# kwea123/ngp_pl

Measured on AMD Instinct MI355X. Metric: train rays/sec (800x800 Lego-like, 8192 rays/batch/GPU, full step incl. optimizer), higher is better.
Workload: dtype f16/f32

## Files before the change

### ngp_pl_amd/_lib.py

```python
import contextlib
import ctypes as C
import os

import torch

_HERE = os.path.dirname(os.path.abspath(__file__))
LIB_PATH = os.environ.get("NGP_HIP_LIB") or os.path.join(_HERE, "csrc", "libngp_hip.so")

P = C.c_void_p
I = C.c_int
F = C.c_float
L = C.c_int64

NGP_MAX_LEVELS = 16


class GridMeta(C.Structure):
    _fields_ = [("n_levels", C.c_int32), ("n_features", C.c_int32),
                ("offset", C.c_uint32 * (NGP_MAX_LEVELS + 1)),
                ("resolution", C.c_uint32 * NGP_MAX_LEVELS),
                ("scale", C.c_float * NGP_MAX_LEVELS)]


class StepperConfig(C.Structure):
# ... 209 lines not shown


def call(name, *args):
    rc = getattr(lib(), name)(*args)
    if name in _COUNT_QUERIES:
        return rc
    if rc != 0:
        kind = {-1: "NGP_EINVAL (bad argument)", -2: "NGP_EUNSUP (unsupported configuration)",
                -3: "NGP_ETIMEOUT (a device result did not arrive within NGP_SPIN_TIMEOUT_S)"}.get(rc, "hipError_t %d" % rc)
        if rc == -4:
            kind = "NGP_ECOMM (%s)" % (lib().ngp_comm_last_error() or b"?").decode(errors="replace")
        raise NgpError("%s failed: %s" % (name, kind))
    return 0


_FIELD_BWD_USES_H = None


def field_bwd_uses_h():
    global _FIELD_BWD_USES_H
    if _FIELD_BWD_USES_H is None:
        _FIELD_BWD_USES_H = bool(call("ngp_field_bwd_uses_h"))
    return _FIELD_BWD_USES_H


SPIN_TIMEOUT_S = float(os.environ.get("NGP_SPIN_TIMEOUT_S", "30"))


class DeviceTimeout(NgpError):
    """A host poll on a device result ran out of time: the kernel named in the message did not finish."""
# ... 77 lines not shown
```

### ngp_pl_amd/build.py

```python
import os
import subprocess
import sys
from concurrent.futures import ThreadPoolExecutor

HERE = os.path.dirname(os.path.abspath(__file__))
CSRC = os.path.join(HERE, "csrc")
LIB = os.path.join(CSRC, "libngp_hip.so")
SOURCES = ["march.hip", "composite.hip", "hashgrid.hip", "mlp.hip", "optim.hip", "occupancy.hip", "hashgrid_bwd_binned.hip", "stepper.hip", "comm.hip"]
HEADERS = ["ngp_common.h", "hashgrid_common.h", "loss_common.h", "comm.h", "adam_common.h", os.path.join("..", "..", "include", "ngp_hip.h")]
ARCH = "gfx950"
HIPCC = os.environ.get("HIPCC", "/opt/rocm/bin/hipcc")
CFLAGS = ["--offload-arch=" + ARCH, "-O3", "-std=c++17", "-fPIC", "-fvisibility=hidden",
          "-fhip-fp32-correctly-rounded-divide-sqrt", "-Wno-unused-result"]
EXTRA = {"mlp.hip": ["-mllvm", "-amdgpu-mfma-vgpr-form"]}
MESH_LIB = os.path.join(CSRC, "libngp_mesh.so")
MESH_SOURCES = [os.path.join("mesh", "mesh.hip")]
MESH_HEADERS = [os.path.join("mesh", "mc_tables.h"), os.path.join("..", "..", "include", "ngp_mesh.h")]
MESH_CFLAGS = ["-ffp-contract=off"]
MESHFILTER_LIB = os.path.join(CSRC, "libngp_meshfilter.so")
MESHFILTER_SOURCES = [os.path.join("meshfilter", "meshfilter.hip")]
MESHFILTER_HEADERS = ["mesh_compact.h", os.path.join("..", "..", "include", "ngp_meshfilter.h")]
MESHCULL_LIB = os.path.join(CSRC, "libngp_meshcull.so")
MESHCULL_SOURCES = [os.path.join("meshcull", "meshcull.hip")]
MESHCULL_HEADERS = ["mesh_compact.h", "mesh_camera.h", "mesh_raster.h", os.path.join("..", "..", "include", "ngp_meshcull.h")]
MESHCULL_CFLAGS = ["-ffp-contract=off"]
MESHSIMPLIFY_LIB = os.path.join(CSRC, "libngp_meshsimplify.so")
MESHSIMPLIFY_SOURCES = [os.path.join("meshsimplify", "meshsimplify.hip")]
MESHSIMPLIFY_HEADERS = ["mesh_compact.h", os.path.join("..", "..", "include", "ngp_meshsimplify.h")]
MESHSIMPLIFY_CFLAGS = ["-ffp-contract=off"]
# ... 55 lines not shown

def _plan(sources, headers, extra, force):
    hdrs = [os.path.join(CSRC, h) for h in headers]
    objs, jobs = [], []
    for src in sources:
        s = os.path.join(CSRC, src)
        o = os.path.join(CSRC, src.replace(".hip", ".o"))
        objs.append(o)
        if force or _stale(o, [s, os.path.abspath(__file__)] + hdrs):
            jobs.append([HIPCC] + CFLAGS + extra(src) + ["-c", s, "-o", o])
    return objs, jobs


def build(force=False, verbose=False):
    objs, jobs = _plan(SOURCES, HEADERS, lambda src: EXTRA.get(src, []), force)
    mesh_objs, mesh_jobs = _plan(MESH_SOURCES, MESH_HEADERS, lambda src: MESH_CFLAGS, force)
    filter_objs, filter_jobs = _plan(MESHFILTER_SOURCES, MESHFILTER_HEADERS, lambda src: [], force)
    cull_objs, cull_jobs = _plan(MESHCULL_SOURCES, MESHCULL_HEADERS, lambda src: MESHCULL_CFLAGS, force)
    simplify_objs, simplify_jobs = _plan(MESHSIMPLIFY_SOURCES, MESHSIMPLIFY_HEADERS, lambda src: MESHSIMPLIFY_CFLAGS, force)
    tsdf_objs, tsdf_jobs = _plan(MESHTSDF_SOURCES, MESHTSDF_HEADERS, lambda src: MESHTSDF_CFLAGS, force)
    smooth_objs, smooth_jobs = _plan(MESHSMOOTH_SOURCES, MESHSMOOTH_HEADERS, lambda src: MESHSMOOTH_CFLAGS, force)
    tex_objs, tex_jobs = _plan(MESHTEX_SOURCES, MESHTEX_HEADERS, lambda src: MESHTEX_CFLAGS, force)
    metrics_objs, metrics_jobs = _plan(METRICS_SOURCES, METRICS_HEADERS, lambda src: METRICS_CFLAGS, force)
    dist_objs, dist_jobs = _plan(MESHDIST_SOURCES, MESHDIST_HEADERS, lambda src: MESHDIST_CFLAGS, force)
    quadric_objs, quadric_jobs = _plan(MESHQUADRIC_SOURCES, MESHQUADRIC_HEADERS, lambda src: MESHQUADRIC_CFLAGS, force)
    decimate_objs, decimate_jobs = _plan(MESHDECIMATE_SOURCES, MESHDECIMATE_HEADERS, lambda src: MESHDECIMATE_CFLAGS, force)
    atlas_objs, atlas_jobs = _plan(MESHATLAS_SOURCES, MESHATLAS_HEADERS, lambda src: MESHATLAS_CFLAGS, force)
    photo_objs, photo_jobs = _plan(MESHPHOTO_SOURCES, MESHPHOTO_HEADERS, lambda src: MESHPHOTO_CFLAGS, force)
    normal_objs, normal_jobs = _plan(MESHNORMAL_SOURCES, MESHNORMAL_HEADERS, lambda src: MESHNORMAL_CFLAGS, force)
    todo = (jobs + mesh_jobs + filter_jobs + cull_jobs + simplify_jobs + tsdf_jobs + smooth_jobs + tex_jobs + metrics_jobs + dist_jobs
            + quadric_jobs + decimate_jobs + atlas_jobs + photo_jobs + normal_jobs)
    if todo:
        if verbose:
            print("[ngp_pl_amd.build] compiling %d HIP sources for %s" % (len(todo), ARCH))
        with ThreadPoolExecutor(max_workers=min(len(todo), os.cpu_count() or 1)) as ex:
            list(ex.map(_run, todo))
    for lib, o, changed in ((LIB, objs, jobs), (MESH_LIB, mesh_objs, mesh_jobs), (MESHFILTER_LIB, filter_objs, filter_jobs),
                            (MESHCULL_LIB, cull_objs, cull_jobs), (MESHSIMPLIFY_LIB, simplify_objs, simplify_jobs),
                            (MESHTSDF_LIB, tsdf_objs, tsdf_jobs), (MESHSMOOTH_LIB, smooth_objs, smooth_jobs),
                            (MESHTEX_LIB, tex_objs, tex_jobs), (METRICS_LIB, metrics_objs, metrics_jobs),
                            (MESHDIST_LIB, dist_objs, dist_jobs), (MESHQUADRIC_LIB, quadric_objs, quadric_jobs),
                            (MESHDECIMATE_LIB, decimate_objs, decimate_jobs), (MESHATLAS_LIB, atlas_objs, atlas_jobs),
                            (MESHPHOTO_LIB, photo_objs, photo_jobs), (MESHNORMAL_LIB, normal_objs, normal_jobs)):
        if force or changed or _stale(lib, o):
            _run([HIPCC, "--offload-arch=" + ARCH, "-shared", "-fPIC"] + o + ["-o", lib])
            if verbose:
                print("[ngp_pl_amd.build] linked", lib)
    return LIB


if __name__ == "__main__":
    build(force="--force" in sys.argv, verbose=True)
# ... 1 lines not shown
```

### ngp_pl_amd/csrc/composite.hip

```cpp
#pragma clang fp contract(off)

#include "ngp_common.h"
#include "loss_common.h"

namespace {

__device__ __forceinline__ float wave_incl_prod(float v, int lane) {
#pragma unroll
    for (int o = 1; o < 64; o <<= 1) { const float u = __shfl_up(v, o, 64); if (lane >= o) v *= u; }
    return v;
}
__device__ __forceinline__ float wave_incl_sum(float v, int lane) {
#pragma unroll
    for (int o = 1; o < 64; o <<= 1) { const float u = __shfl_up(v, o, 64); if (lane >= o) v += u; }
    return v;
}

struct ChunkT { float a, T_before, T_after; bool live; uint64_t stop; };
__device__ __forceinline__ ChunkT chunk_transmittance(float sigma, float delta, bool valid, float T_carry, float thr, int lane) {
    ChunkT c;
    c.a = valid ? 1.0f - __expf(-sigma * delta) : 0.0f;
    const float incl = wave_incl_prod(1.0f - c.a, lane);
    const float excl = __shfl_up(incl, 1, 64);
    c.T_before = T_carry * (lane == 0 ? 1.0f : excl);
    c.T_after = T_carry * incl;
    c.stop = __ballot(valid && c.T_after <= thr);
    const int first_stop = c.stop ? __ffsll((long long)c.stop) - 1 : 64;
    c.live = valid && lane <= first_stop && (c.T_before > thr);
    return c;
}

struct FwTail {
    const float* gt; const float* bg; float lambda_o, grad_scale;
    float* loss; float* sq_err; float* dL_drgb; float* dL_dopacity;
    int32_t* n_active; float* row_loss; float* row_sq;
    int32_t* n_active_host;
    float* rgb_out;
};
// ... 13 lines not shown
    int base = 0;
    for (; base < N && !stopped; base += 64) {
        const int k = base + lane;
        const bool valid = k < N;
        const size_t s = (size_t)start + (valid ? k : 0);
        const float sigma = valid ? sigmas[s] : 0.f, delta = valid ? deltas[s] : 0.f;
        const ChunkT c = chunk_transmittance(sigma, delta, valid, T_carry, T_threshold, lane);
        const float w = c.live ? c.a * c.T_before : 0.0f;
        if (valid) ws[s] = w;
        if (c.live) {
            R += w * rgbs[3 * s]; G += w * rgbs[3 * s + 1]; B += w * rgbs[3 * s + 2];
            D += w * ts[s]; O += w;
        }
        samples += __popcll(__ballot(c.live && c.T_after > T_threshold));
        stopped = c.stop != 0ull;
        T_carry = __shfl(c.T_after, 63, 64);
    }
    for (int k = base + lane; k < N; k += 64) ws[(size_t)start + k] = 0.0f;
    R = ngp_wave_sum(R); G = ngp_wave_sum(G); B = ngp_wave_sum(B); D = ngp_wave_sum(D); O = ngp_wave_sum(O);
    if (lane == 0) {
        rgb[3 * ray_idx] = R; rgb[3 * ray_idx + 1] = G; rgb[3 * ray_idx + 2] = B;
        depth[ray_idx] = D; opacity[ray_idx] = O;
        total_samples[ray_idx] = samples;
        if (n_active_per_ray) n_active_per_ray[n] = min(N, samples + 1);
        if (tail && tail->gt) {
            const float c[3] = {R, G, B};
            const float g[3] = {tail->gt[3 * ray_idx], tail->gt[3 * ray_idx + 1], tail->gt[3 * ray_idx + 2]};
            float d_rgb[3], d_o, l = 0.f, se = 0.f;
            nerf_loss_ray(O, c, g, tail->bg, tail->lambda_o, tail->grad_scale, 1.0f / (float)n_rays, 1.0f / (3.0f * (float)n_rays),
                          d_rgb, d_o, l, se);
            tail->dL_drgb[3 * ray_idx] = d_rgb[0]; tail->dL_drgb[3 * ray_idx + 1] = d_rgb[1]; tail->dL_drgb[3 * ray_idx + 2] = d_rgb[2];
// ... 99 lines not shown
composite_train_fw_kernel(const float* __restrict__ sigmas, const float* __restrict__ rgbs,
                          const float* __restrict__ deltas, const float* __restrict__ ts,
                          const int64_t* __restrict__ rays_a, float T_threshold, int n_rays,
                          int64_t* __restrict__ total_samples, float* __restrict__ opacity,
                          float* __restrict__ depth, float* __restrict__ rgb, float* __restrict__ ws,
                          int32_t* __restrict__ n_active_per_ray, FwTail tail) {
    const int n = (blockIdx.x * blockDim.x + threadIdx.x) >> 6;
    const int lane = threadIdx.x & 63;
    if (n >= n_rays) return;
    composite_fw_ray(sigmas, rgbs, deltas, ts, rays_a, T_threshold, n, lane, total_samples, opacity, depth, rgb, ws,
                     n_active_per_ray, LOSS ? &tail : nullptr, n_rays);
}

struct BwTail { const float* row_loss; const float* row_sq; float* loss; float* sq_err; int32_t* n_active; int32_t* n_active_host;
                const float* bg; int blend; };
__device__ __forceinline__ int wave_sum_int(int v) {
#pragma unroll
    for (int o = 32; o > 0; o >>= 1) v += __shfl_xor(v, o, 64);
    return v;
}

template <bool FUSED_TAIL>
__global__ void __launch_bounds__(256)
composite_train_bw_kernel(const float* __restrict__ dL_dopacity, const float* __restrict__ dL_ddepth,
                          const float* __restrict__ dL_drgb, const float* __restrict__ dL_dws,
                          const float* __restrict__ sigmas, const float* __restrict__ rgbs,
                          const float* __restrict__ ws, const float* __restrict__ deltas,
                          const float* __restrict__ ts, const int64_t* __restrict__ rays_a,
                          const float* __restrict__ opacity, const float* __restrict__ depth,
                          const float* __restrict__ rgb, float T_threshold, int n_rays,
                          float* __restrict__ dL_dsigmas, float* __restrict__ dL_drgbs,
                          const int32_t* __restrict__ ray_offsets, int32_t* __restrict__ active_idx,
                          const float* __restrict__ xyzs, float* __restrict__ x_active, BwTail tail) {
    const int n = (blockIdx.x * blockDim.x + threadIdx.x) >> 6;
    const int lane = threadIdx.x & 63;
// ... 4 lines not shown
        const int tid = threadIdx.x, wave = tid >> 6;
        const int row0 = 4 * (int)blockIdx.x;
        int4 v[8];
#pragma unroll
        for (int q = 0; q < 8; ++q) {
            const int i = 4 * tid + 1024 * q;
            v[q] = i < row0 ? *reinterpret_cast<const int4*>(ray_offsets + i) : make_int4(0, 0, 0, 0);
        }
        int acc = 0;
#pragma unroll
        for (int q = 0; q < 8; ++q) acc += (v[q].x + v[q].y) + (v[q].z + v[q].w);
        for (int i = 4 * tid + 8192; i < row0; i += 1024) {
            const int4 a = *reinterpret_cast<const int4*>(ray_offsets + i);
            acc += (a.x + a.y) + (a.z + a.w);
        }
        acc = wave_sum_int(acc);
        if (lane == 0) s_part[wave] = acc;
        __syncthreads();
        const int wg_prefix = (s_part[0] + s_part[1]) + (s_part[2] + s_part[3]);
        int own[4];
#pragma unroll
        for (int w = 0; w < 4; ++w) own[w] = (row0 + w < n_rays) ? ray_offsets[row0 + w] : 0;
        a_off = wg_prefix;
#pragma unroll
        for (int w = 0; w < 4; ++w) if (w < wave) a_off += own[w];
        if (blockIdx.x == gridDim.x - 1 && tid == 0) {
            const int total = wg_prefix + ((own[0] + own[1]) + (own[2] + own[3]));
            *tail.n_active = total;
            if (tail.n_active_host) *tail.n_active_host = total;
        }
        if (blockIdx.x == 0 && tail.row_loss != nullptr) {
// ... 50 lines not shown
                const float T = c.T_after;
                dr = gR * w; dg = gG * w; db = gB * w;
                ds = delta * (gR * (cr * T - (R - r)) + gG * (cg * T - (G - g)) + gB * (cb * T - (B - b)) +
                              gO * (1 - O) + gD * (tk * T - (D - d)) + T * gw - (P_total - P));
            }
            dL_dsigmas[s] = ds; dL_drgbs[3 * s] = dr; dL_drgbs[3 * s + 1] = dg; dL_drgbs[3 * s + 2] = db;
            if (active_idx && c.live) {
                active_idx[a_off + k] = (int32_t)s;
                if (x_active) {
                    float* __restrict__ xo = x_active + 3 * (size_t)(a_off + k);
                    xo[0] = xyzs[3 * s]; xo[1] = xyzs[3 * s + 1]; xo[2] = xyzs[3 * s + 2];
                }
            }
        }
        stopped = c.stop != 0ull;
        T_carry = __shfl(c.T_after, 63, 64);
        r0 = __shfl(r, 63, 64); g0 = __shfl(g, 63, 64); b0 = __shfl(b, 63, 64); d0 = __shfl(d, 63, 64); P0 = __shfl(P, 63, 64);
    }
    for (int k = base + lane; k < N; k += 64) {
        const size_t s = (size_t)start + k;
        dL_dsigmas[s] = 0.f; dL_drgbs[3 * s] = 0.f; dL_drgbs[3 * s + 1] = 0.f; dL_drgbs[3 * s + 2] = 0.f;
    }
}

__global__ void __launch_bounds__(64)
composite_test_fw_kernel(const float* __restrict__ sigmas, const float* __restrict__ rgbs,
                         const float* __restrict__ deltas, const float* __restrict__ ts,
                         int64_t* __restrict__ alive, float T_threshold,
                         const int32_t* __restrict__ n_eff, int n_alive, int n_samples,
                         float* __restrict__ opacity, float* __restrict__ depth, float* __restrict__ rgb) {
    const int n = blockIdx.x * blockDim.x + threadIdx.x;
    if (n >= n_alive) return;
// ... 276 lines not shown
```

### ngp_pl_amd/csrc/hashgrid.hip

```cpp
#include "hashgrid_common.h"
#include <hip/hip_fp16.h>
#include <cstdlib>
#include <cstring>

using namespace ngp_grid;

namespace {

__device__ __forceinline__ bool map_block(int n_levels, int n_chunks, int& level, int& chunk) {
    const int b = blockIdx.x;
    const int xcd = b & 7, q = b >> 3;
    const int slot = q / n_chunks;
    chunk = q - slot * n_chunks;
    if (n_levels == 16) level = (slot == 0) ? xcd : 15 - xcd;
    else level = xcd + 8 * slot;
    return level < n_levels;
}

struct FwdMap {
    int32_t end[8][16];
    uint32_t piece[8][16];
    uint32_t magic[8][16];
    int32_t blocks_per_xcd;
};
// ... 71 lines not shown
        n_samples = min(*n_dev, n_samples);
        if (chunk * SPT * 256 >= n_samples) return;
    }
    const uint32_t res = meta.resolution[level];
    const uint32_t size = meta.offset[level + 1] - meta.offset[level];
    const half2_t* __restrict__ tab = table + meta.offset[level];
    const Box box = load_box(xyz_min, xyz_max);
    const bool hashed = level_is_hashed(res, size);
    const float scale = meta.scale[level];
    static_assert(SPT == 1, "one sample per thread: 2 or 4 measured the same (the kernel is bound by gather transactions)");
    {
        const int i = chunk * 256 + threadIdx.x, lane = threadIdx.x & 63;
        const bool ok = i < n_samples;
        uint32_t p[3]; float f[3];
        cell_of(x, box, (size_t)(ok ? i : n_samples - 1), scale, p, f);
        const uint32_t q0 = __shfl_up(p[0], 1, 64), q1 = __shfl_up(p[1], 1, 64), q2 = __shfl_up(p[2], 1, 64);
        const bool first = lane == 0 || p[0] != q0 || p[1] != q1 || p[2] != q2;
        const unsigned long long firsts = __ballot(first);
        const int src = 63 - __builtin_clzll(firsts & ((2ull << lane) - 1ull));
        half2_t v[8];
#pragma unroll
        for (int c = 0; c < 8; ++c) { v[c][0] = (_Float16)0; v[c][1] = (_Float16)0; }
        if (first) {
            if (hashed) gather_corners<true>(tab, p, res, size, v);
            else gather_corners<false>(tab, p, res, size, v);
        }
        float o0 = 0.f, o1 = 0.f;
#pragma unroll
        for (int c = 0; c < 8; ++c) {
            const half2_t u = lane_read(v[c], src);
            const float w = corner_weight(c, f);
// ... 14 lines not shown
    if (!map_block(meta.n_levels, n_chunks, level, chunk)) return;
    if (n_list_dev != nullptr) n_list = min(*n_list_dev, n_list);
    const uint32_t res = meta.resolution[level];
    const uint32_t size = meta.offset[level + 1] - meta.offset[level];
    const half2_t* __restrict__ tab = table + meta.offset[level];
    const Box box = load_box(xyz_min, xyz_max);
    const bool hashed = level_is_hashed(res, size);
    const float scale = meta.scale[level];
    const int lane = threadIdx.x & 63;
    for (int jw = chunk * 256 + (int)(threadIdx.x & ~63u); jw < n_list; jw += n_chunks * 256) {
        const int j = jw + lane;
        const int i = j < n_list ? list[j] : -1;
        const bool valid = (unsigned)i < (unsigned)n_samples;
        uint32_t p[3]; float f[3];
        cell_of(x, box, (size_t)(valid ? i : 0), scale, p, f);
        const uint32_t q0 = __shfl_up(p[0], 1, 64), q1 = __shfl_up(p[1], 1, 64), q2 = __shfl_up(p[2], 1, 64);
        const bool prev_valid = __shfl_up((int)valid, 1, 64) != 0;
        const bool first = valid && (lane == 0 || !prev_valid || p[0] != q0 || p[1] != q1 || p[2] != q2);
        const unsigned long long firsts = __ballot(first);
        const unsigned long long upto = firsts & ((2ull << lane) - 1ull);
        const int src = upto ? 63 - __builtin_clzll(upto) : lane;
        half2_t v[8];
#pragma unroll
        for (int c = 0; c < 8; ++c) { v[c][0] = (_Float16)0; v[c][1] = (_Float16)0; }
        if (first) {
            if (hashed) gather_corners<true>(tab, p, res, size, v);
            else gather_corners<false>(tab, p, res, size, v);
        }
        float o0 = 0.f, o1 = 0.f;
#pragma unroll
        for (int c = 0; c < 8; ++c) {
            const half2_t u = lane_read(v[c], src);
// ... 554 lines not shown
```

### ngp_pl_amd/csrc/hashgrid_bwd_binned.hip

```cpp
#include "hashgrid_common.h"
#include <hip/hip_fp16.h>

using namespace ngp_grid;

namespace {

#ifndef NGP_SLICE2
#define NGP_SLICE2 6912
#endif
#ifndef NGP_APPLY_WGS
#define NGP_APPLY_WGS 256
#endif
constexpr uint32_t SLICE2 = NGP_SLICE2;
constexpr int MAX_SLICES = ((1 << 19) + SLICE2 - 1) / SLICE2 + 4;
constexpr float FIX_SCALE = 16777216.0f;
constexpr int BIN_THREADS = 512;
#ifndef NGP_BIN_SPT
#define NGP_BIN_SPT 2
#endif
constexpr int BIN_SPT = NGP_BIN_SPT;
constexpr int CHUNK = BIN_THREADS * BIN_SPT;
constexpr int CHUNK_SLOTS = CHUNK * 8;
constexpr int MAX_CHUNKS = 4608;
#ifndef NGP_APPLY_THREADS
// ... 99 lines not shown
                    }
                }
            }
        }
    }
#pragma unroll
    for (int t = 0; t < BIN_SPT; ++t)
#pragma unroll
        for (int q = 0; q < 8; ++q) if (q < n_mine[t] && sid[t][q] >= 0) loc[t][q] = atomicAdd(&s_cnt[sid[t][q]], 1);
    __syncthreads();
    if (threadIdx.x < 64) {
        int run = 0;
        for (int b0 = 0; b0 < ns; b0 += 64) {
            const int i = b0 + (int)threadIdx.x;
            const int v = (i < ns) ? s_cnt[i] : 0;
            int incl = v;
#pragma unroll
            for (int o = 1; o < 64; o <<= 1) { const int u = __shfl_up(incl, o, 64); if ((int)threadIdx.x >= o) incl += u; }
            if (i < ns) s_pre[i] = run + incl - v;
            run += __shfl(incl, 63, 64);
        }
        if (threadIdx.x == 0) s_pre[ns] = run;
    }
    __syncthreads();
    int32_t* __restrict__ slot = ws.pool + plan.pool_off[level] + (size_t)chunk * CHUNK_SLOTS * plan.entry_words[level];
    {
#pragma unroll
        for (int t = 0; t < BIN_SPT; ++t)
#pragma unroll
            for (int q = 0; q < 8; ++q) if (q < n_mine[t] && sid[t][q] >= 0) s_stage[s_pre[sid[t][q]] + loc[t][q]] = (jj[t] << 2) | tag[t][q];
        __syncthreads();
        const int total = s_pre[ns];
        for (int i = threadIdx.x; i < total; i += BIN_THREADS) slot[i] = s_stage[i];
    }
    for (int i = threadIdx.x; i < ns; i += BIN_THREADS) dir[(size_t)i * n_chunks] = (s_pre[i] << 16) | s_cnt[i];
// ... 249 lines not shown
        const uint32_t lo = (uint32_t)slice * SLICE2;
        const uint32_t len = min(SLICE2, size - lo);
        const int* s_dir = s_dir2[it & 1];
#ifdef NGP_BIN_TIMING
        if (tid == 0) ws.timing[4 * task + 1] = (long long)wall_clock64();
#endif
        const half2_t* __restrict__ g_level = dfeats + (size_t)level * n_samples;
        const int32_t* __restrict__ pool_level = ws.pool + plan.pool_off[level];
        if (level_is_hashed(res, size)) {
            apply_segments_hashed<NGP_APPLY_B>(lds, lo, len, res, size, meta.scale[level], x, box, g_level, active, pool_level, s_dir, n_chunks, part, K);
        }
        else if (NGP_DENSE_RUNS) apply_segments_dense_runs<NGP_DENSE_B>(lds, lo, len, res, size, meta.scale[level], x, box, g_level, active, pool_level, s_dir, n_chunks, part, K);
        else apply_segments_dense<4>(lds, lo, len, res, size, meta.scale[level], x, box, g_level, active, pool_level, s_dir, n_chunks, part, K);
#if NGP_DIR_BY_WAVE0
        if (tid < 64) {
            const int nt0 = __shfl(next_task, 0, 64);
            if (tid == 0) s_task[(it + 1) & 1] = nt0;
            if (nt0 < task_end) {
                const int32_t* __restrict__ dn = dir_row(nt0);
                int* __restrict__ dst = s_dir2[(it + 1) & 1];
                for (int c0 = 0; c0 < n_chunks; c0 += 64 * 8) {
                    int v[8];
#pragma unroll
                    for (int q = 0; q < 8; ++q) { const int c = c0 + q * 64 + tid; v[q] = c < n_chunks ? dn[c] : 0; }
#pragma unroll
                    for (int q = 0; q < 8; ++q) { const int c = c0 + q * 64 + tid; if (c < n_chunks) dst[c] = v[q]; }
                }
            }
        }
#else
        if (tid == 0) s_task[(it + 1) & 1] = next_task;
// ... 270 lines not shown
```

### ngp_pl_amd/csrc/march.hip

```cpp
#pragma clang fp contract(off)

#include <cstdlib>
#include <chrono>
#include <type_traits>
#include "ngp_common.h"

#define NGP_SQRT3 1.73205080757f

namespace {

__device__ __forceinline__ float2 aabb_hit(float ox, float oy, float oz, float ix, float iy, float iz,
                                           float cx, float cy, float cz, float hx, float hy, float hz) {
    const float tminx = (cx - hx - ox) * ix, tmaxx = (cx + hx - ox) * ix;
    const float tminy = (cy - hy - oy) * iy, tmaxy = (cy + hy - oy) * iy;
    const float tminz = (cz - hz - oz) * iz, tmaxz = (cz + hz - oz) * iz;
    const float t1 = fmaxf(fmaxf(fminf(tminx, tmaxx), fminf(tminy, tmaxy)), fminf(tminz, tmaxz));
    const float t2 = fminf(fminf(fmaxf(tminx, tmaxx), fmaxf(tminy, tmaxy)), fmaxf(tminz, tmaxz));
    if (t1 > t2) return make_float2(-1.0f, -1.0f);
    return make_float2(t1, t2);
}

__device__ __forceinline__ float2 sphere_hit(float ox, float oy, float oz, float dx, float dy, float dz,
                                             float cx, float cy, float cz, float radius) {
    const float cox = ox - cx, coy = oy - cy, coz = oz - cz;
// ... 624 lines not shown
    if (s > 0) hits_t[2 * r] = t_resume;
    n_eff[n] = s;
    for (int k = s; k < n_samples; ++k) write_sample(xyzs, dirs, deltas, ts, base + k, 0.f, 0.f, 0.f, 0.f, 0.f, 0.f, 0.f, 0.f);
}

__global__ void __launch_bounds__(256)
compact_alive_kernel(const int64_t* __restrict__ alive_in, const int32_t* __restrict__ n_eff, int n,
                     int64_t* __restrict__ alive_out, int32_t* __restrict__ count, int64_t* __restrict__ total) {
    const int i = blockIdx.x * blockDim.x + threadIdx.x;
    const int lane = threadIdx.x & 63;
    const int64_t a = (i < n) ? alive_in[i] : -1;
    const bool keep = a >= 0;
    const unsigned long long m = __ballot(keep);
    int base = 0;
    if (lane == 0 && m) base = atomicAdd(count, __popcll(m));
    base = __shfl(base, 0, 64);
    if (keep) alive_out[base + __popcll(m & ((1ull << lane) - 1ull))] = a;
    if (total != nullptr) {
        const int e = ngp_wave_sum_i32((i < n && n_eff != nullptr) ? n_eff[i] : 0);
        if (lane == 0 && e) atomicAdd(reinterpret_cast<unsigned long long*>(total), (unsigned long long)e);
    }
}

MarchParams make_march_params(const uint8_t* bitfield, int cascades, int grid_size, float scale,
                              float scale_for_dt, float esf, int max_samples) {
    MarchParams p;
    p.bitfield = bitfield; p.cascades = cascades; p.grid_size = grid_size; p.scale = scale; p.esf = esf;
    p.dt_lo = NGP_SQRT3 / max_samples;
    p.dt_hi = NGP_SQRT3 * 2 * scale_for_dt / grid_size;
    p.bound0 = fminf(scalbnf(1.0f, -1), scale);
    p.bound0_inv = 1 / p.bound0;
// ... 115 lines not shown
                ++probes;
                float x, y, z, dt, t_next;
                if (march_probe<SIMPLE>(ray, p, t, x, y, z, dt, t_next, nullptr, any, hop_slack)) {
                    s_t[s * 64 + lane] = t;
                    t += dt; ++s;
                } else {
                    t = t_next;
                }
            }
            hits[2 * r] = t;
            const int e = emitted[r] + s;
            emitted[r] = e;
            if (e >= max_samples_total) flags = RENDER_RETIRE;
        }
    }
    int incl = s;
#pragma unroll
    for (int o = 1; o < 64; o <<= 1) {
        const int v = __shfl_up(incl, o, 64);
        if (lane >= o) incl += v;
    }
    const int total = __shfl(incl, 63, 64);
    int base = 0;
    if (lane == 63 && total > 0) base = atomicAdd(&plan->m, total);
    base = __shfl(base, 63, 64);
    if (active) { offsets[n] = base + incl - s; n_eff[n] = s | flags; }
    s_incl[lane] = incl;
    s_ray[lane] = ray.ox; s_ray[64 + lane] = ray.oy; s_ray[128 + lane] = ray.oz;
    s_ray[192 + lane] = ray.dx; s_ray[256 + lane] = ray.dy; s_ray[320 + lane] = ray.dz;
    wave_lds_fence();
    for (int j = lane; j < total; j += 64) {
        int lo = 0;
#pragma unroll
        for (int step = 32; step > 0; step >>= 1)
            if (s_incl[lo + step - 1] <= j) lo += step;
        const int k = j - (lo ? s_incl[lo - 1] : 0);
        const float t = s_t[k * 64 + lo];
        const float ox = s_ray[lo], oy = s_ray[64 + lo], oz = s_ray[128 + lo];
        const float dx = s_ray[192 + lo], dy = s_ray[256 + lo], dz = s_ray[320 + lo];
        write_sample(xyzs, dirs, deltas, ts, (size_t)base + j, ox, oy, oz, dx, dy, dz, t, SIMPLE ? p.dt_lo : calc_dt(t, p));
// ... 640 lines not shown
```

### ngp_pl_amd/csrc/ngp_common.h

```cpp
#pragma once
#include <hip/hip_runtime.h>
#include <stdint.h>
#include "../../include/ngp_hip.h"
#include "ngp_internal.h"

#define NGP_WAVE 64

#define NGP_CHECK_PTR(p) do { if ((p) == nullptr) return NGP_EINVAL; } while (0)
#define NGP_LAUNCH_RESULT() ((int)hipGetLastError())

static inline hipStream_t ngp_stream(ngp_stream_t s) { return reinterpret_cast<hipStream_t>(s); }
static inline int ngp_div_up(long long a, long long b) { return (int)((a + b - 1) / b); }

__device__ __forceinline__ uint32_t ngp_expand_bits(uint32_t v) {
    v = (v * 0x00010001u) & 0xFF0000FFu;
    v = (v * 0x00000101u) & 0x0F00F00Fu;
    v = (v * 0x00000011u) & 0xC30C30C3u;
    v = (v * 0x00000005u) & 0x49249249u;
    return v;
}
__device__ __forceinline__ uint32_t ngp_morton3D(uint32_t x, uint32_t y, uint32_t z) {
    return ngp_expand_bits(x) | (ngp_expand_bits(y) << 1) | (ngp_expand_bits(z) << 2);
}
__device__ __forceinline__ uint32_t ngp_compact_bits(uint32_t x) {
// ... 2 lines not shown
    x = (x | (x >> 4)) & 0x0F00F00Fu;
    x = (x | (x >> 8)) & 0xFF0000FFu;
    x = (x | (x >> 16)) & 0x0000FFFFu;
    return x;
}

__device__ __forceinline__ uint32_t ngp_pcg_hash(uint32_t v) {
    uint32_t state = v * 747796405u + 2891336453u;
    uint32_t word = ((state >> ((state >> 28u) + 4u)) ^ state) * 277803737u;
    return (word >> 22u) ^ word;
}
__device__ __forceinline__ uint32_t ngp_rng_key(uint32_t seed_lo, uint32_t seed_hi, uint32_t i) {
    return ngp_pcg_hash(ngp_pcg_hash(seed_lo ^ ngp_pcg_hash(i)) + seed_hi);
}

__device__ __forceinline__ float ngp_wave_sum(float v) {
#pragma unroll
    for (int o = 32; o > 0; o >>= 1) v += __shfl_xor(v, o, 64);
    return v;
}

__device__ __forceinline__ int ngp_wave_sum_i32(int v) {
#pragma unroll
    for (int o = 32; o > 0; o >>= 1) v += __shfl_xor(v, o, 64);
    return v;
}

template <int ITEMS>
__device__ __forceinline__ int ngp_block_scan_tile(const int (&v)[ITEMS], int* s_wave, int* s_carry) {
    const int tid = threadIdx.x, lane = tid & 63, wave = tid >> 6;
    int mine = 0;
#pragma unroll
    for (int k = 0; k < ITEMS; ++k) mine += v[k];
    int incl = mine;
#pragma unroll
    for (int o = 1; o < 64; o <<= 1) {
        const int u = __shfl_up(incl, o, 64);
        if (lane >= o) incl += u;
    }
    if (lane == 63) s_wave[wave] = incl;
    __syncthreads();
    int off = *s_carry;
    for (int w = 0; w < wave; ++w) off += s_wave[w];
    __syncthreads();
    if (tid == (int)blockDim.x - 1) *s_carry = off + incl;
    return off + incl - mine;
}
```

### ngp_pl_amd/csrc/occupancy.hip

```cpp
#include "ngp_common.h"

namespace {

__device__ __forceinline__ uint32_t occ_hash(uint32_t v) {
    uint32_t state = v * 747796405u + 2891336453u;
    uint32_t word = ((state >> ((state >> 28u) + 4u)) ^ state) * 277803737u;
    return (word >> 22u) ^ word;
}
__device__ __forceinline__ float u01(uint32_t r) { return (float)(r >> 8) * (1.0f / 16777216.0f); }

__global__ void __launch_bounds__(256)
occ_words_kernel(const float* __restrict__ grid, float threshold, int n_words,
                 unsigned long long* __restrict__ words, int32_t* __restrict__ counts) {
    const int w = (blockIdx.x * blockDim.x + threadIdx.x) >> 6;
    const int lane = threadIdx.x & 63;
    if (w >= n_words) return;
    const unsigned long long m = __ballot(grid[(size_t)w * 64 + lane] > threshold);
    if (lane == 0) { words[w] = m; counts[w] = __popcll(m); }
}

__device__ __forceinline__ int wave_incl_scan(int v, int lane) {
#pragma unroll
    for (int o = 1; o < 64; o <<= 1) {
        const int u = __shfl_up(v, o, 64);
        if (lane >= o) v += u;
    }
    return v;
}
__global__ void __launch_bounds__(1024)
occ_scan_kernel(const int32_t* __restrict__ counts, int n, int32_t* __restrict__ prefix) {
    __shared__ int s_wave[16];
    const int tid = threadIdx.x, lane = tid & 63, wave = tid >> 6;
    const int n4 = n >> 2;
    const int run = ((n4 + 15) / 16 + 63) / 64 * 64;
    const int begin = min(wave * run, n4), end = min(begin + run, n4);
    const int4* c4 = reinterpret_cast<const int4*>(counts);
    int sum = 0;
    for (int g = begin + lane; g < end; g += 64) { const int4 v = c4[g]; sum += (v.x + v.y) + (v.z + v.w); }
    sum = wave_incl_scan(sum, lane);
    if (lane == 63) s_wave[wave] = sum;
    __syncthreads();
    int carry = 0;
    for (int w = 0; w < wave; ++w) carry += s_wave[w];
    for (int g0 = begin; g0 < end; g0 += 64) {
        const int g = g0 + lane;
        int4 v = {0, 0, 0, 0};
        if (g < end) v = c4[g];
        const int local = (v.x + v.y) + (v.z + v.w);
        const int incl = wave_incl_scan(local, lane);
        int4 o; o.x = carry + incl - local; o.y = o.x + v.x; o.z = o.y + v.y; o.w = o.z + v.z;
        if (g < end) reinterpret_cast<int4*>(prefix)[g] = o;
        carry += __shfl(incl, 63, 64);
    }
    if (tid == 1023) {
        int total = carry;
        for (int i = 4 * n4; i < n; ++i) { prefix[i] = total; total += counts[i]; }
        prefix[n] = total;
    }
}

__device__ __forceinline__ int select_bit(unsigned long long m, int r) {
    int pos = 0;
#pragma unroll
    for (int width = 32; width > 0; width >>= 1) {
        const unsigned long long low = (m >> pos) & ((1ull << width) - 1ull);
        const int c = __popcll(low);
        if (r >= c) { r -= c; pos += width; }
// ... 58 lines not shown
    s_hist[threadIdx.x] = 0;
    __syncthreads();
    for (int i = begin + threadIdx.x; i < end; i += 1024) atomicAdd(&s_hist[((uint32_t)drawn[(size_t)half * M + i]) >> shift], 1);
    __syncthreads();
    hist[(size_t)blockIdx.x * OCC_BUCKETS + threadIdx.x] = s_hist[threadIdx.x];
}

__global__ void __launch_bounds__(1024)
occ_hist_scan_kernel(int32_t* __restrict__ hist, int M) {
    __shared__ int s_wave[16];
    const int b = threadIdx.x, lane = b & 63, wave = b >> 6;
    int32_t* h = hist + (size_t)blockIdx.x * OCC_SORT_WGS * OCC_BUCKETS;
    int total = 0;
#pragma unroll 16
    for (int w = 0; w < OCC_SORT_WGS; ++w) total += h[w * OCC_BUCKETS + b];
    const int incl = wave_incl_scan(total, lane);
    if (lane == 63) s_wave[wave] = incl;
    __syncthreads();
    int run = (int)blockIdx.x * M + incl - total;
    for (int w = 0; w < wave; ++w) run += s_wave[w];
    for (int w0 = 0; w0 < OCC_SORT_WGS; w0 += 16) {
        int c[16];
#pragma unroll
        for (int k = 0; k < 16; ++k) c[k] = h[(w0 + k) * OCC_BUCKETS + b];
#pragma unroll
        for (int k = 0; k < 16; ++k) { h[(w0 + k) * OCC_BUCKETS + b] = run; run += c[k]; }
    }
}

__global__ void __launch_bounds__(1024)
occ_place_kernel(const int32_t* __restrict__ drawn, int M, int shift, const int32_t* __restrict__ offsets, int grid_size,
// ... 198 lines not shown
```

Before: 24.11 million.

## Replace ds_bpermute wave shuffles with DPP, permlane swaps and readlane

Adds a wave_ops.h header that implements wave shift-up, xor, broadcast, inclusive scan and sum using DPP row ops, gfx950 permlane16/32 swaps and readlane in place of __shfl-based LDS permutes. The header is then used in compositing, hashgrid, binned backward, march and occupancy kernels. The aim is to cut the latency and LDS traffic of cross-lane communication in scans and reductions. A debug library that compares each op against the reference shuffle is also added. If any DPP control or mask encoding is wrong, results could be silently incorrect.

```diff
diff --git a/ngp_pl_amd/_lib.py b/ngp_pl_amd/_lib.py
--- a/ngp_pl_amd/_lib.py
+++ b/ngp_pl_amd/_lib.py
@@ -247,6 +247,32 @@
     return 0
 
 
+WAVEOPS_LIB_PATH = os.path.join(_HERE, "csrc", "libngp_waveops.so")
+WAVE_OP_KINDS = {"shift_up_1": 0, "shift_up_2": 1, "shift_up_4": 2, "shift_up_8": 3, "shift_up_16": 4, "shift_up_32": 5,
+                 "xor_1": 6, "xor_2": 7, "xor_4": 8, "xor_8": 9, "xor_16": 10, "xor_32": 11, "bcast_0": 12, "bcast_63": 13,
+                 "incl_prod": 14, "incl_sum": 15, "incl_scan_i32": 16, "sum_f32": 17, "sum_i32": 18}
+_waveops = None
+
+
+def debug_wave_ops(kind, words):
+    global _waveops
+    if _waveops is None:
+        if not os.path.exists(WAVEOPS_LIB_PATH):
+            raise RuntimeError("libngp_waveops.so is missing (%s): run `python -m ngp_pl_amd.build`" % WAVEOPS_LIB_PATH)
+        h = C.CDLL(WAVEOPS_LIB_PATH)
+        h.ngp_debug_wave_ops.argtypes = [I, P, I, P, P, P]
+        h.ngp_debug_wave_ops.restype = I
+        _waveops = h
+    require_cuda(words)
+    if words.dtype != torch.int32 or words.dim() != 2 or words.shape[1] != 64:
+        raise ValueError("words: an (n_waves, 64) int32 tensor")
+    out_new, out_ref = torch.empty_like(words), torch.empty_like(words)
+    rc = _waveops.ngp_debug_wave_ops(WAVE_OP_KINDS[kind], ptr(words), words.shape[0], ptr(out_new), ptr(out_ref), stream())
+    if rc != 0:
+        raise NgpError("ngp_debug_wave_ops(%s) failed: %d" % (kind, rc))
+    return out_new, out_ref
+
+
 _FIELD_BWD_USES_H = None
 
 
diff --git a/ngp_pl_amd/build.py b/ngp_pl_amd/build.py
--- a/ngp_pl_amd/build.py
+++ b/ngp_pl_amd/build.py
@@ -7,12 +7,15 @@
 CSRC = os.path.join(HERE, "csrc")
 LIB = os.path.join(CSRC, "libngp_hip.so")
 SOURCES = ["march.hip", "composite.hip", "hashgrid.hip", "mlp.hip", "optim.hip", "occupancy.hip", "hashgrid_bwd_binned.hip", "stepper.hip", "comm.hip"]
-HEADERS = ["ngp_common.h", "hashgrid_common.h", "loss_common.h", "comm.h", "adam_common.h", os.path.join("..", "..", "include", "ngp_hip.h")]
+HEADERS = ["ngp_common.h", "wave_ops.h", "hashgrid_common.h", "loss_common.h", "comm.h", "adam_common.h", os.path.join("..", "..", "include", "ngp_hip.h")]
 ARCH = "gfx950"
 HIPCC = os.environ.get("HIPCC", "/opt/rocm/bin/hipcc")
 CFLAGS = ["--offload-arch=" + ARCH, "-O3", "-std=c++17", "-fPIC", "-fvisibility=hidden",
           "-fhip-fp32-correctly-rounded-divide-sqrt", "-Wno-unused-result"]
 EXTRA = {"mlp.hip": ["-mllvm", "-amdgpu-mfma-vgpr-form"]}
+WAVEOPS_LIB = os.path.join(CSRC, "libngp_waveops.so")
+WAVEOPS_SOURCES = ["wave_ops_debug.hip"]
+WAVEOPS_HEADERS = ["wave_ops.h"]
 MESH_LIB = os.path.join(CSRC, "libngp_mesh.so")
 MESH_SOURCES = [os.path.join("mesh", "mesh.hip")]
 MESH_HEADERS = [os.path.join("mesh", "mc_tables.h"), os.path.join("..", "..", "include", "ngp_mesh.h")]
@@ -98,6 +101,7 @@
 
 def build(force=False, verbose=False):
     objs, jobs = _plan(SOURCES, HEADERS, lambda src: EXTRA.get(src, []), force)
+    waveops_objs, waveops_jobs = _plan(WAVEOPS_SOURCES, WAVEOPS_HEADERS, lambda src: [], force)
     mesh_objs, mesh_jobs = _plan(MESH_SOURCES, MESH_HEADERS, lambda src: MESH_CFLAGS, force)
     filter_objs, filter_jobs = _plan(MESHFILTER_SOURCES, MESHFILTER_HEADERS, lambda src: [], force)
     cull_objs, cull_jobs = _plan(MESHCULL_SOURCES, MESHCULL_HEADERS, lambda src: MESHCULL_CFLAGS, force)
@@ -112,14 +116,14 @@
     atlas_objs, atlas_jobs = _plan(MESHATLAS_SOURCES, MESHATLAS_HEADERS, lambda src: MESHATLAS_CFLAGS, force)
     photo_objs, photo_jobs = _plan(MESHPHOTO_SOURCES, MESHPHOTO_HEADERS, lambda src: MESHPHOTO_CFLAGS, force)
     normal_objs, normal_jobs = _plan(MESHNORMAL_SOURCES, MESHNORMAL_HEADERS, lambda src: MESHNORMAL_CFLAGS, force)
-    todo = (jobs + mesh_jobs + filter_jobs + cull_jobs + simplify_jobs + tsdf_jobs + smooth_jobs + tex_jobs + metrics_jobs + dist_jobs
+    todo = (jobs + waveops_jobs + mesh_jobs + filter_jobs + cull_jobs + simplify_jobs + tsdf_jobs + smooth_jobs + tex_jobs + metrics_jobs + dist_jobs
             + quadric_jobs + decimate_jobs + atlas_jobs + photo_jobs + normal_jobs)
     if todo:
         if verbose:
             print("[ngp_pl_amd.build] compiling %d HIP sources for %s" % (len(todo), ARCH))
         with ThreadPoolExecutor(max_workers=min(len(todo), os.cpu_count() or 1)) as ex:
             list(ex.map(_run, todo))
-    for lib, o, changed in ((LIB, objs, jobs), (MESH_LIB, mesh_objs, mesh_jobs), (MESHFILTER_LIB, filter_objs, filter_jobs),
+    for lib, o, changed in ((LIB, objs, jobs), (WAVEOPS_LIB, waveops_objs, waveops_jobs), (MESH_LIB, mesh_objs, mesh_jobs), (MESHFILTER_LIB, filter_objs, filter_jobs),
                             (MESHCULL_LIB, cull_objs, cull_jobs), (MESHSIMPLIFY_LIB, simplify_objs, simplify_jobs),
                             (MESHTSDF_LIB, tsdf_objs, tsdf_jobs), (MESHSMOOTH_LIB, smooth_objs, smooth_jobs),
                             (MESHTEX_LIB, tex_objs, tex_jobs), (METRICS_LIB, metrics_objs, metrics_jobs),
diff --git a/ngp_pl_amd/csrc/composite.hip b/ngp_pl_amd/csrc/composite.hip
--- a/ngp_pl_amd/csrc/composite.hip
+++ b/ngp_pl_amd/csrc/composite.hip
@@ -2,26 +2,16 @@
 
 #include "ngp_common.h"
 #include "loss_common.h"
+#include "wave_ops.h"
 
 namespace {
-
-__device__ __forceinline__ float wave_incl_prod(float v, int lane) {
-#pragma unroll
-    for (int o = 1; o < 64; o <<= 1) { const float u = __shfl_up(v, o, 64); if (lane >= o) v *= u; }
-    return v;
-}
-__device__ __forceinline__ float wave_incl_sum(float v, int lane) {
-#pragma unroll
-    for (int o = 1; o < 64; o <<= 1) { const float u = __shfl_up(v, o, 64); if (lane >= o) v += u; }
-    return v;
-}
 
 struct ChunkT { float a, T_before, T_after; bool live; uint64_t stop; };
 __device__ __forceinline__ ChunkT chunk_transmittance(float sigma, float delta, bool valid, float T_carry, float thr, int lane) {
     ChunkT c;
     c.a = valid ? 1.0f - __expf(-sigma * delta) : 0.0f;
     const float incl = wave_incl_prod(1.0f - c.a, lane);
-    const float excl = __shfl_up(incl, 1, 64);
+    const float excl = wave_shift_up<1>(incl);
     c.T_before = T_carry * (lane == 0 ? 1.0f : excl);
     c.T_after = T_carry * incl;
     c.stop = __ballot(valid && c.T_after <= thr);
@@ -65,7 +55,7 @@
         }
         samples += __popcll(__ballot(c.live && c.T_after > T_threshold));
         stopped = c.stop != 0ull;
-        T_carry = __shfl(c.T_after, 63, 64);
+        T_carry = wave_bcast<63>(c.T_after);
     }
     for (int k = base + lane; k < N; k += 64) ws[(size_t)start + k] = 0.0f;
     R = ngp_wave_sum(R); G = ngp_wave_sum(G); B = ngp_wave_sum(B); D = ngp_wave_sum(D); O = ngp_wave_sum(O);
@@ -195,11 +185,6 @@
 
 struct BwTail { const float* row_loss; const float* row_sq; float* loss; float* sq_err; int32_t* n_active; int32_t* n_active_host;
                 const float* bg; int blend; };
-__device__ __forceinline__ int wave_sum_int(int v) {
-#pragma unroll
-    for (int o = 32; o > 0; o >>= 1) v += __shfl_xor(v, o, 64);
-    return v;
-}
 
 template <bool FUSED_TAIL>
 __global__ void __launch_bounds__(256)
@@ -234,7 +219,7 @@
             const int4 a = *reinterpret_cast<const int4*>(ray_offsets + i);
             acc += (a.x + a.y) + (a.z + a.w);
         }
-        acc = wave_sum_int(acc);
+        acc = ngp_wave_sum_i32(acc);
         if (lane == 0) s_part[wave] = acc;
         __syncthreads();
         const int wg_prefix = (s_part[0] + s_part[1]) + (s_part[2] + s_part[3]);
@@ -315,8 +300,8 @@
             }
         }
         stopped = c.stop != 0ull;
-        T_carry = __shfl(c.T_after, 63, 64);
-        r0 = __shfl(r, 63, 64); g0 = __shfl(g, 63, 64); b0 = __shfl(b, 63, 64); d0 = __shfl(d, 63, 64); P0 = __shfl(P, 63, 64);
+        T_carry = wave_bcast<63>(c.T_after);
+        r0 = wave_bcast<63>(r); g0 = wave_bcast<63>(g); b0 = wave_bcast<63>(b); d0 = wave_bcast<63>(d); P0 = wave_bcast<63>(P);
     }
     for (int k = base + lane; k < N; k += 64) {
         const size_t s = (size_t)start + k;
diff --git a/ngp_pl_amd/csrc/hashgrid.hip b/ngp_pl_amd/csrc/hashgrid.hip
--- a/ngp_pl_amd/csrc/hashgrid.hip
+++ b/ngp_pl_amd/csrc/hashgrid.hip
@@ -109,7 +109,7 @@
         const bool ok = i < n_samples;
         uint32_t p[3]; float f[3];
         cell_of(x, box, (size_t)(ok ? i : n_samples - 1), scale, p, f);
-        const uint32_t q0 = __shfl_up(p[0], 1, 64), q1 = __shfl_up(p[1], 1, 64), q2 = __shfl_up(p[2], 1, 64);
+        const uint32_t q0 = wave_shift_up<1>(p[0]), q1 = wave_shift_up<1>(p[1]), q2 = wave_shift_up<1>(p[2]);
         const bool first = lane == 0 || p[0] != q0 || p[1] != q1 || p[2] != q2;
         const unsigned long long firsts = __ballot(first);
         const int src = 63 - __builtin_clzll(firsts & ((2ull << lane) - 1ull));
@@ -154,8 +154,8 @@
         const bool valid = (unsigned)i < (unsigned)n_samples;
         uint32_t p[3]; float f[3];
         cell_of(x, box, (size_t)(valid ? i : 0), scale, p, f);
-        const uint32_t q0 = __shfl_up(p[0], 1, 64), q1 = __shfl_up(p[1], 1, 64), q2 = __shfl_up(p[2], 1, 64);
-        const bool prev_valid = __shfl_up((int)valid, 1, 64) != 0;
+        const uint32_t q0 = wave_shift_up<1>(p[0]), q1 = wave_shift_up<1>(p[1]), q2 = wave_shift_up<1>(p[2]);
+        const bool prev_valid = wave_shift_up<1>((int)valid) != 0;
         const bool first = valid && (lane == 0 || !prev_valid || p[0] != q0 || p[1] != q1 || p[2] != q2);
         const unsigned long long firsts = __ballot(first);
         const unsigned long long upto = firsts & ((2ull << lane) - 1ull);
diff --git a/ngp_pl_amd/csrc/hashgrid_bwd_binned.hip b/ngp_pl_amd/csrc/hashgrid_bwd_binned.hip
--- a/ngp_pl_amd/csrc/hashgrid_bwd_binned.hip
+++ b/ngp_pl_amd/csrc/hashgrid_bwd_binned.hip
@@ -137,11 +137,9 @@
         for (int b0 = 0; b0 < ns; b0 += 64) {
             const int i = b0 + (int)threadIdx.x;
             const int v = (i < ns) ? s_cnt[i] : 0;
-            int incl = v;
-#pragma unroll
-            for (int o = 1; o < 64; o <<= 1) { const int u = __shfl_up(incl, o, 64); if ((int)threadIdx.x >= o) incl += u; }
+            const int incl = wave_incl_scan(v);
             if (i < ns) s_pre[i] = run + incl - v;
-            run += __shfl(incl, 63, 64);
+            run += wave_bcast<63>(incl);
         }
         if (threadIdx.x == 0) s_pre[ns] = run;
     }
@@ -421,7 +419,7 @@
         else apply_segments_dense<4>(lds, lo, len, res, size, meta.scale[level], x, box, g_level, active, pool_level, s_dir, n_chunks, part, K);
 #if NGP_DIR_BY_WAVE0
         if (tid < 64) {
-            const int nt0 = __shfl(next_task, 0, 64);
+            const int nt0 = wave_bcast<0>(next_task);
             if (tid == 0) s_task[(it + 1) & 1] = nt0;
             if (nt0 < task_end) {
                 const int32_t* __restrict__ dn = dir_row(nt0);
diff --git a/ngp_pl_amd/csrc/march.hip b/ngp_pl_amd/csrc/march.hip
--- a/ngp_pl_amd/csrc/march.hip
+++ b/ngp_pl_amd/csrc/march.hip
@@ -662,7 +662,7 @@
     const unsigned long long m = __ballot(keep);
     int base = 0;
     if (lane == 0 && m) base = atomicAdd(count, __popcll(m));
-    base = __shfl(base, 0, 64);
+    base = wave_bcast<0>(base);
     if (keep) alive_out[base + __popcll(m & ((1ull << lane) - 1ull))] = a;
     if (total != nullptr) {
         const int e = ngp_wave_sum_i32((i < n && n_eff != nullptr) ? n_eff[i] : 0);
@@ -808,16 +808,11 @@
             if (e >= max_samples_total) flags = RENDER_RETIRE;
         }
     }
-    int incl = s;
-#pragma unroll
-    for (int o = 1; o < 64; o <<= 1) {
-        const int v = __shfl_up(incl, o, 64);
-        if (lane >= o) incl += v;
-    }
-    const int total = __shfl(incl, 63, 64);
+    const int incl = wave_incl_scan(s);
+    const int total = wave_bcast<63>(incl);
     int base = 0;
     if (lane == 63 && total > 0) base = atomicAdd(&plan->m, total);
-    base = __shfl(base, 63, 64);
+    base = wave_bcast<63>(base);
     if (active) { offsets[n] = base + incl - s; n_eff[n] = s | flags; }
     s_incl[lane] = incl;
     s_ray[lane] = ray.ox; s_ray[64 + lane] = ray.oy; s_ray[128 + lane] = ray.oz;
diff --git a/ngp_pl_amd/csrc/ngp_common.h b/ngp_pl_amd/csrc/ngp_common.h
--- a/ngp_pl_amd/csrc/ngp_common.h
+++ b/ngp_pl_amd/csrc/ngp_common.h
@@ -3,6 +3,7 @@
 #include <stdint.h>
 #include "../../include/ngp_hip.h"
 #include "ngp_internal.h"
+#include "wave_ops.h"
 
 #define NGP_WAVE 64
 
@@ -40,17 +41,8 @@
     return ngp_pcg_hash(ngp_pcg_hash(seed_lo ^ ngp_pcg_hash(i)) + seed_hi);
 }
 
-__device__ __forceinline__ float ngp_wave_sum(float v) {
-#pragma unroll
-    for (int o = 32; o > 0; o >>= 1) v += __shfl_xor(v, o, 64);
-    return v;
-}
-
-__device__ __forceinline__ int ngp_wave_sum_i32(int v) {
-#pragma unroll
-    for (int o = 32; o > 0; o >>= 1) v += __shfl_xor(v, o, 64);
-    return v;
-}
+__device__ __forceinline__ float ngp_wave_sum(float v) { return wave_sum(v); }
+__device__ __forceinline__ int ngp_wave_sum_i32(int v) { return wave_sum(v); }
 
 template <int ITEMS>
 __device__ __forceinline__ int ngp_block_scan_tile(const int (&v)[ITEMS], int* s_wave, int* s_carry) {
@@ -58,12 +50,7 @@
     int mine = 0;
 #pragma unroll
     for (int k = 0; k < ITEMS; ++k) mine += v[k];
-    int incl = mine;
-#pragma unroll
-    for (int o = 1; o < 64; o <<= 1) {
-        const int u = __shfl_up(incl, o, 64);
-        if (lane >= o) incl += u;
-    }
+    const int incl = wave_incl_scan(mine);
     if (lane == 63) s_wave[wave] = incl;
     __syncthreads();
     int off = *s_carry;
diff --git a/ngp_pl_amd/csrc/occupancy.hip b/ngp_pl_amd/csrc/occupancy.hip
--- a/ngp_pl_amd/csrc/occupancy.hip
+++ b/ngp_pl_amd/csrc/occupancy.hip
@@ -19,14 +19,6 @@
     if (lane == 0) { words[w] = m; counts[w] = __popcll(m); }
 }
 
-__device__ __forceinline__ int wave_incl_scan(int v, int lane) {
-#pragma unroll
-    for (int o = 1; o < 64; o <<= 1) {
-        const int u = __shfl_up(v, o, 64);
-        if (lane >= o) v += u;
-    }
-    return v;
-}
 __global__ void __launch_bounds__(1024)
 occ_scan_kernel(const int32_t* __restrict__ counts, int n, int32_t* __restrict__ prefix) {
     __shared__ int s_wave[16];
@@ -37,7 +29,7 @@
     const int4* c4 = reinterpret_cast<const int4*>(counts);
     int sum = 0;
     for (int g = begin + lane; g < end; g += 64) { const int4 v = c4[g]; sum += (v.x + v.y) + (v.z + v.w); }
-    sum = wave_incl_scan(sum, lane);
+    sum = wave_incl_scan(sum);
     if (lane == 63) s_wave[wave] = sum;
     __syncthreads();
     int carry = 0;
@@ -47,10 +39,10 @@
         int4 v = {0, 0, 0, 0};
         if (g < end) v = c4[g];
         const int local = (v.x + v.y) + (v.z + v.w);
-        const int incl = wave_incl_scan(local, lane);
+        const int incl = wave_incl_scan(local);
         int4 o; o.x = carry + incl - local; o.y = o.x + v.x; o.z = o.y + v.y; o.w = o.z + v.z;
         if (g < end) reinterpret_cast<int4*>(prefix)[g] = o;
-        carry += __shfl(incl, 63, 64);
+        carry += wave_bcast<63>(incl);
     }
     if (tid == 1023) {
         int total = carry;
@@ -139,7 +131,7 @@
     int total = 0;
 #pragma unroll 16
     for (int w = 0; w < OCC_SORT_WGS; ++w) total += h[w * OCC_BUCKETS + b];
-    const int incl = wave_incl_scan(total, lane);
+    const int incl = wave_incl_scan(total);
     if (lane == 63) s_wave[wave] = incl;
     __syncthreads();
     int run = (int)blockIdx.x * M + incl - total;
diff --git a/ngp_pl_amd/csrc/wave_ops.h b/ngp_pl_amd/csrc/wave_ops.h
--- /dev/null
+++ b/ngp_pl_amd/csrc/wave_ops.h
@@ -0,0 +1,136 @@
+#pragma once
+#include <hip/hip_runtime.h>
+#include <stdint.h>
+
+namespace wave_detail {
+
+template <typename T> __device__ __forceinline__ int to_bits(T v) {
+    static_assert(sizeof(T) == 4, "32-bit values only");
+    return __builtin_bit_cast(int, v);
+}
+template <typename T> __device__ __forceinline__ T from_bits(int b) { return __builtin_bit_cast(T, b); }
+
+template <int CTRL, int ROW_MASK = 0xF, int BANK_MASK = 0xF>
+__device__ __forceinline__ int dpp(int old, int src) {
+    return __builtin_amdgcn_update_dpp(old, src, CTRL, ROW_MASK, BANK_MASK, false);
+}
+constexpr int QUAD_IDENTITY = 0xE4;
+
+__device__ __forceinline__ void swap16(int v, int& even, int& odd) {
+    const auto r = __builtin_amdgcn_permlane16_swap((unsigned)v, (unsigned)v, false, false);
+    even = (int)r[0]; odd = (int)r[1];
+}
+__device__ __forceinline__ void swap32(int a, int b, int& lo, int& hi) {
+    const auto r = __builtin_amdgcn_permlane32_swap((unsigned)a, (unsigned)b, false, false);
+    lo = (int)r[0]; hi = (int)r[1];
+}
+
+template <int O> __device__ __forceinline__ int shift_up_bits(int v);
+template <> __device__ __forceinline__ int shift_up_bits<1>(int v) { return dpp<0x138>(v, v); }
+template <> __device__ __forceinline__ int shift_up_bits<2>(int v) { return shift_up_bits<1>(shift_up_bits<1>(v)); }
+template <> __device__ __forceinline__ int shift_up_bits<4>(int v) { return shift_up_bits<2>(shift_up_bits<2>(v)); }
+template <> __device__ __forceinline__ int shift_up_bits<32>(int v) {
+    int lo, hi;
+    swap32(v, v, lo, hi);
+    return lo;
+}
+template <> __device__ __forceinline__ int shift_up_bits<16>(int v) {
+    int even, odd, lo, hi;
+    swap16(v, even, odd);
+    swap32(odd, odd, lo, hi);
+    return dpp<QUAD_IDENTITY, 0x4>(even, lo);
+}
+template <> __device__ __forceinline__ int shift_up_bits<8>(int v) {
+    const int same_row = dpp<0x118>(v, v);
+    return dpp<0x128, 0xF, 0x3>(same_row, shift_up_bits<16>(v));
+}
+
+template <int O> __device__ __forceinline__ int xor_bits(int v);
+template <> __device__ __forceinline__ int xor_bits<1>(int v) { return dpp<0xB1>(v, v); }
+template <> __device__ __forceinline__ int xor_bits<2>(int v) { return dpp<0x4E>(v, v); }
+template <> __device__ __forceinline__ int xor_bits<4>(int v) {
+    const int t = dpp<0x104, 0xF, 0x5>(v, v);
+    return dpp<0x114, 0xF, 0xA>(t, v);
+}
+template <> __device__ __forceinline__ int xor_bits<8>(int v) { return dpp<0x128>(v, v); }
+template <> __device__ __forceinline__ int xor_bits<16>(int v) {
+    int even, odd;
+    swap16(v, even, odd);
+    return dpp<QUAD_IDENTITY, 0x5>(even, odd);
+}
+template <> __device__ __forceinline__ int xor_bits<32>(int v) {
+    int lo, hi;
+    swap32(v, v, lo, hi);
+    return dpp<QUAD_IDENTITY, 0x3>(lo, hi);
+}
+
+__device__ __forceinline__ int lane_id() { return (int)__builtin_amdgcn_mbcnt_hi(~0u, __builtin_amdgcn_mbcnt_lo(~0u, 0u)); }
+
+}
+
+template <int O, typename T> __device__ __forceinline__ T wave_shift_up(T v) {
+    return wave_detail::from_bits<T>(wave_detail::shift_up_bits<O>(wave_detail::to_bits(v)));
+}
+template <int O, typename T> __device__ __forceinline__ T wave_shift_up_ref(T v) { return __shfl_up(v, O, 64); }
+
+template <int O, typename T> __device__ __forceinline__ T wave_xor(T v) {
+    return wave_detail::from_bits<T>(wave_detail::xor_bits<O>(wave_detail::to_bits(v)));
+}
+template <int O, typename T> __device__ __forceinline__ T wave_xor_ref(T v) { return __shfl_xor(v, O, 64); }
+
+template <int LANE, typename T> __device__ __forceinline__ T wave_bcast(T v) {
+    static_assert(LANE >= 0 && LANE < 64, "lane of a wave64");
+    return wave_detail::from_bits<T>(__builtin_amdgcn_readlane(wave_detail::to_bits(v), LANE));
+}
+template <int LANE, typename T> __device__ __forceinline__ T wave_bcast_ref(T v) { return __shfl(v, LANE, 64); }
+
+#define NGP_WAVE_SCAN_STEP(O, OP) { const float u = wave_shift_up<O>(v); if (lane >= O) v OP u; }
+__device__ __forceinline__ float wave_incl_prod(float v, int lane) {
+    NGP_WAVE_SCAN_STEP(1, *=) NGP_WAVE_SCAN_STEP(2, *=) NGP_WAVE_SCAN_STEP(4, *=)
+    NGP_WAVE_SCAN_STEP(8, *=) NGP_WAVE_SCAN_STEP(16, *=) NGP_WAVE_SCAN_STEP(32, *=)
+    return v;
+}
+__device__ __forceinline__ float wave_incl_sum(float v, int lane) {
+    NGP_WAVE_SCAN_STEP(1, +=) NGP_WAVE_SCAN_STEP(2, +=) NGP_WAVE_SCAN_STEP(4, +=)
+    NGP_WAVE_SCAN_STEP(8, +=) NGP_WAVE_SCAN_STEP(16, +=) NGP_WAVE_SCAN_STEP(32, +=)
+    return v;
+}
+#undef NGP_WAVE_SCAN_STEP
+__device__ __forceinline__ float wave_incl_prod_ref(float v, int lane) {
+#pragma unroll
+    for (int o = 1; o < 64; o <<= 1) { const float u = __shfl_up(v, o, 64); if (lane >= o) v *= u; }
+    return v;
+}
+__device__ __forceinline__ float wave_incl_sum_ref(float v, int lane) {
+#pragma unroll
+    for (int o = 1; o < 64; o <<= 1) { const float u = __shfl_up(v, o, 64); if (lane >= o) v += u; }
+    return v;
+}
+
+__device__ __forceinline__ int wave_incl_scan(int v) {
+    using wave_detail::dpp;
+    v += dpp<0x111>(0, v);
+    v += dpp<0x112>(0, v);
+    v += dpp<0x114>(0, v);
+    v += dpp<0x118>(0, v);
+    v += dpp<0x142, 0xA>(0, v);
+    v += dpp<0x143, 0xC>(0, v);
+    return v;
+}
+__device__ __forceinline__ int wave_incl_scan_ref(int v) {
+    const int lane = wave_detail::lane_id();
+#pragma unroll
+    for (int o = 1; o < 64; o <<= 1) { const int u = __shfl_up(v, o, 64); if (lane >= o) v += u; }
+    return v;
+}
+
+template <typename T> __device__ __forceinline__ T wave_sum(T v) {
+    v += wave_xor<32>(v); v += wave_xor<16>(v); v += wave_xor<8>(v);
+    v += wave_xor<4>(v); v += wave_xor<2>(v); v += wave_xor<1>(v);
+    return v;
+}
+template <typename T> __device__ __forceinline__ T wave_sum_ref(T v) {
+#pragma unroll
+    for (int o = 32; o > 0; o >>= 1) v += __shfl_xor(v, o, 64);
+    return v;
+}
diff --git a/ngp_pl_amd/csrc/wave_ops_debug.hip b/ngp_pl_amd/csrc/wave_ops_debug.hip
--- /dev/null
+++ b/ngp_pl_amd/csrc/wave_ops_debug.hip
@@ -0,0 +1,61 @@
+#include <hip/hip_runtime.h>
+#include <stdint.h>
+#include "wave_ops.h"
+
+namespace {
+
+enum Kind {
+    SHIFT_UP_1 = 0, SHIFT_UP_2, SHIFT_UP_4, SHIFT_UP_8, SHIFT_UP_16, SHIFT_UP_32,
+    XOR_1 = 6, XOR_2, XOR_4, XOR_8, XOR_16, XOR_32,
+    BCAST_0 = 12, BCAST_63,
+    INCL_PROD = 14, INCL_SUM, INCL_SCAN_I32, SUM_F32, SUM_I32,
+    N_KINDS
+};
+
+template <int KIND> __device__ __forceinline__ void apply(int x, int lane, int& a, int& b) {
+    const float f = __builtin_bit_cast(float, x);
+    float fa = 0.f, fb = 0.f;
+    bool is_float = false;
+    if constexpr (KIND >= SHIFT_UP_1 && KIND <= SHIFT_UP_32) { constexpr int O = 1 << (KIND - SHIFT_UP_1); a = wave_shift_up<O>(x); b = wave_shift_up_ref<O>(x); }
+    else if constexpr (KIND >= XOR_1 && KIND <= XOR_32) { constexpr int O = 1 << (KIND - XOR_1); a = wave_xor<O>(x); b = wave_xor_ref<O>(x); }
+    else if constexpr (KIND == BCAST_0) { a = wave_bcast<0>(x); b = wave_bcast_ref<0>(x); }
+    else if constexpr (KIND == BCAST_63) { a = wave_bcast<63>(x); b = wave_bcast_ref<63>(x); }
+    else if constexpr (KIND == INCL_PROD) { fa = wave_incl_prod(f, lane); fb = wave_incl_prod_ref(f, lane); is_float = true; }
+    else if constexpr (KIND == INCL_SUM) { fa = wave_incl_sum(f, lane); fb = wave_incl_sum_ref(f, lane); is_float = true; }
+    else if constexpr (KIND == INCL_SCAN_I32) { a = wave_incl_scan(x); b = wave_incl_scan_ref(x); }
+    else if constexpr (KIND == SUM_F32) { fa = wave_sum(f); fb = wave_sum_ref(f); is_float = true; }
+    else { a = wave_sum(x); b = wave_sum_ref(x); }
+    if (is_float) { a = __builtin_bit_cast(int, fa); b = __builtin_bit_cast(int, fb); }
+}
+
+template <int KIND>
+__global__ void __launch_bounds__(256)
+wave_ops_kernel(const int* __restrict__ in, int n_waves, int* __restrict__ out_new, int* __restrict__ out_ref) {
+    const int wave = (int)((blockIdx.x * blockDim.x + threadIdx.x) >> 6), lane = (int)(threadIdx.x & 63);
+    if (wave >= n_waves) return;
+    const size_t i = (size_t)wave * 64 + lane;
+    int a, b;
+    apply<KIND>(in[i], lane, a, b);
+    out_new[i] = a; out_ref[i] = b;
+}
+
+template <int KIND>
+int launch(int kind, const int* in, int n_waves, int* out_new, int* out_ref, hipStream_t stream) {
+    if constexpr (KIND < N_KINDS) {
+        if (kind != KIND) return launch<KIND + 1>(kind, in, n_waves, out_new, out_ref, stream);
+        hipLaunchKernelGGL(wave_ops_kernel<KIND>, dim3((unsigned)((n_waves + 3) / 4)), dim3(256), 0, stream, in, n_waves, out_new, out_ref);
+        return (int)hipGetLastError();
+    }
+    return -1;
+}
+
+}
+
+extern "C" __attribute__((visibility("default")))
+int ngp_debug_wave_ops(int kind, const void* in, int n_waves, void* out_new, void* out_ref, void* stream) {
+    if (kind < 0 || kind >= N_KINDS || n_waves < 0 || n_waves > (1 << 20)) return -1;
+    if (n_waves == 0) return 0;
+    if (in == nullptr || out_new == nullptr || out_ref == nullptr) return -1;
+    return launch<0>(kind, static_cast<const int*>(in), n_waves, static_cast<int*>(out_new), static_cast<int*>(out_ref),
+                     reinterpret_cast<hipStream_t>(stream));
+}
```

After: 23.97 million. Within noise of the previous version (-0.6%).
